# worldfnd/provekit

Hardware: AMD Instinct MI355X
Metric: proofs/sec (noir-r1cs prove hot path, WHIR commit + sumcheck + folding rounds) (higher is better)
Workload: dtype u32x8 (BN254-Fr, 256-bit Montgomery integers); 1 GPU; poseidon-rounds size class: m=21, m_0=20, satisfiable synthetic R1CS (786429 constraints, 1048571 witnesses, a constant term in half of the rows of A and B), batch-2 WHIR commit + zk-sumcheck + 4-round WHIR opening, queries [109, 28, 16, 11]/9, pow_bits [19.0, 16.0, 16.0, 18.0]/11.0 (WhirConfig::new derivation, security 128, ConjectureList), blinding WHIR n=8 queries [122]/31, Skyscraper-sponge tr; launcher=single process

## Files before the change

### provekit_amd/csrc/internal.hpp

```cpp
#pragma once
#include "ctx.hpp"
#include "rng_core.hpp"

namespace pk {

int ensure_scratch(pk_ctx* ctx, size_t bytes);
int ensure_pinned(pk_ctx* ctx);
int ensure_ws(pk_ctx* ctx, size_t bytes);
enum { PK_HOOK_GATE_SPINS = 0, PK_HOOK_GATE_STALL_US = 1, PK_HOOK_RCCL_SAME_DEVICE = 2, PK_HOOK_COUNT = 3 };
long test_hook(int which);
hipError_t wait_stream(int device, hipStream_t stream);
hipError_t wait_ctx(pk_ctx* ctx);
int wait_ctx_rc(pk_ctx* ctx);
int sync_stream(pk_ctx* ctx);
int mail_alloc(pk_ctx* ctx, size_t bytes, void** out);

int comm_rank(const pk_ctx* ctx);
int comm_world(const pk_ctx* ctx);
int comm_all_gather(pk_ctx* ctx, const void* d_send, void* d_recv, size_t bytes_per_rank);
int comm_all_reduce_sum_u64(pk_ctx* ctx, uint64_t* d_buf, size_t count);
int comm_collect_fe(pk_ctx* ctx, int K, uint64_t* host_out);
int red_across_begin(pk_ctx* ctx);
bool comm_collective_pending(const pk_ctx* ctx);
bool comm_rccl(const pk_ctx* ctx);
hipError_t comm_wait(pk_ctx* ctx);
void comm_turn_begin(pk_ctx* ctx);
void comm_turn_end(pk_ctx* ctx);
unsigned long long comm_collectives_issued(const pk_ctx* ctx);
void comm_abort(pk_ctx* ctx);
void comm_release(pk_ctx* ctx);

int leaf_hash_x(pk_ctx* ctx, const uint64_t* d_leaves, size_t n_leaves, size_t width, uint64_t* d_digests, bool scaled_in);
int merkle_top_x(pk_ctx* ctx, uint64_t* d_nodes, size_t top_leaves);
int read_root(pk_ctx* ctx, const uint64_t* d_nodes, size_t n_leaves, uint64_t root[4]);

void ntt_retain_ctx(pk_ctx* ctx);
void ntt_release_ctx(pk_ctx* ctx);
bool ntt_scaled_available(unsigned log_n);
int rs_encode_x(pk_ctx* ctx, const uint64_t* const* d_coeffs, unsigned batch, unsigned n_vars, unsigned log_inv_rate, unsigned fold,
                uint64_t* d_leaves, uint64_t* d_scratch, bool scaled);
int rs_encode_shard_x(pk_ctx* ctx, const uint64_t* const* d_coeffs, unsigned batch, unsigned n_vars, unsigned log_inv_rate, unsigned fold,
                      unsigned shard, unsigned n_shards, uint64_t* d_leaves_local, uint64_t* d_scratch, bool scaled);

int pow_solve_x(pk_ctx* ctx, const uint8_t challenge[32], double bits, uint64_t* nonce, bool striped);

unsigned shard_factor(const pk_ctx* ctx, size_t rows);
size_t commit_scratch_fes(const pk_ctx* ctx, size_t rows, size_t width);
int commit_into(pk_ctx* ctx, const uint64_t* const* d_coeffs, unsigned batch, unsigned n_vars, unsigned log_inv_rate, unsigned fold,
                uint64_t* d_leaves, uint64_t* d_nodes, uint64_t* d_scratch, pk_commit_layout* layout_out);
int open_raw(pk_ctx* ctx, const uint64_t* d_leaves, const uint64_t* d_nodes, size_t n_leaves, size_t width, const pk_commit_layout& lay,
             const uint64_t* indices, size_t k, int canonical_leaves, uint64_t* leaves_out, uint64_t* sibling_digests, uint64_t* auth_paths);

int eval_univariate_multi(pk_ctx* ctx, const uint64_t* const* d_polys, unsigned np, size_t n, const uint64_t z[4], uint64_t* out);
int dot_rows(pk_ctx* ctx, const uint64_t* d_w, size_t row_stride, unsigned nrows, const uint64_t* d_f, const uint64_t* d_g, size_t n, uint64_t* out,
             bool defer = false);
int lincomb2(pk_ctx* ctx, uint64_t* d_out, const uint64_t* d_a, const uint64_t* beta, const uint64_t* d_b, size_t n);
int fold_pairs2(pk_ctx* ctx, const uint64_t* d_v0, uint64_t* d_out0, const uint64_t* d_v1, uint64_t* d_out1, size_t len, const uint64_t* r,
                unsigned gate_seq = 0);
int sumcheck_cubic_launch(pk_ctx* ctx, uint64_t* d_a, uint64_t* d_b, uint64_t* d_c, uint64_t* d_eq, size_t len, const uint64_t* fold_or_null,
                          unsigned gate_seq, unsigned* red_seq_out);
int sumcheck_quadratic_launch(pk_ctx* ctx, const uint64_t* d_f, const uint64_t* d_w, size_t len, const uint64_t* fold_or_null, unsigned gate_seq,
                              uint64_t* d_f_out, uint64_t* d_w_out, int nsums, unsigned* red_seq_out);
void sumcheck_quadratic_from_claim(const uint64_t claim[4], uint64_t out[12]);
int eq_suffix_tables(pk_ctx* ctx, const uint64_t* r, unsigned n, uint64_t* d_out);
int sumcheck_cubic_spliteq_launch(pk_ctx* ctx, uint64_t* d_a, uint64_t* d_b, uint64_t* d_c, const uint64_t* d_level, size_t len,
                                  const uint64_t* fold_or_null, unsigned gate_seq, unsigned* red_seq_out);
void sumcheck_spliteq_correct(const uint64_t P[4], const uint64_t r_i[4], uint64_t out[12]);
void sumcheck_spliteq_advance(uint64_t P[4], const uint64_t r_i[4], const uint64_t alpha_i[4]);
int sumcheck_collect_spin(pk_ctx* ctx, int nsums, unsigned red_seq, uint64_t out[12]);
int sumcheck_collect(pk_ctx* ctx, int nsums, uint64_t out[12]);
unsigned sumcheck_gate_next(pk_ctx* ctx);
void sumcheck_gate_publish(pk_ctx* ctx, unsigned gate_seq, const uint64_t challenge[4]);
int sumcheck_gate_check(pk_ctx* ctx);
void sumcheck_gate_clear(pk_ctx* ctx);

int witness_bounds_strided(pk_ctx* ctx, const pk_r1cs* r, const uint64_t* d_z, unsigned m0, unsigned stride, unsigned offset, uint64_t* d_a,
                           uint64_t* d_b, uint64_t* d_c);
int external_row_range(pk_ctx* ctx, const pk_r1cs* r, const uint64_t* d_eq_alpha, size_t first, size_t last, uint64_t* d_out);

enum { RNG_MASK = 1, RNG_G = 2, RNG_BLIND = 3, RNG_MASK_B = 4, RNG_G_B = 5, RNG_FILL = 6 };
int proof_key(pk_ctx* ctx, const uint8_t* rng_seed32, RngKey& key);
int random_fe(pk_ctx* ctx, uint64_t* d_out, size_t n, const RngKey& key, uint32_t stream);

void witness_program_shape(const pk_witness_program* p, size_t* n_witnesses, size_t* n_challenges, size_t* n_acir);
int witness_phase_shape(const uint8_t* bytes, size_t len, std::vector<uint32_t>& widths, std::vector<uint32_t>& op_counts, std::vector<uint32_t>& blocks_before,
                        std::string& error);

const char* whir_config_error(const pk_whir_config* c);
unsigned blinding_log_len(unsigned m_0);
// ... 8 lines not shown
```

### provekit_amd/csrc/mle.hip

```cpp
#define PK_BASE_PRIO 2
#include "internal.hpp"
#include "fe29.hpp"
#include "reduce.hpp"

using namespace pk;

namespace {

struct fe_arg {
    u32 v[8];
};
__device__ __forceinline__ fe from_arg(const fe_arg& a) {
    fe r;
#pragma unroll
    for (int i = 0; i < 8; i++) r.v[i] = a.v[i];
    return r;
}
inline fe_arg to_arg(const uint64_t* h) {
    fe_arg a;
    memcpy(a.v, h, 32);
    return a;
}

__device__ __forceinline__ fe lds_get(const uint4* lo, const uint4* hi, int i) {
// ... 46 lines not shown
    const int R = 1 << logr;
    const int TILE = R * BT;
    uint4* lo = lds;
    uint4* hi = lds + TILE;
    const size_t vblocks = ((size_t)1 << s) / BT;
    const size_t u = blockIdx.x / vblocks, vb = blockIdx.x % vblocks;
    fe* base = data + (u << (s + logr)) + vb * BT;
    for (int e = threadIdx.x; e < TILE; e += 256) {
        int b = e % BT, r = e / BT;
        const uint4* q = reinterpret_cast<const uint4*>(base + ((size_t)r << s) + b);
        lo[e] = q[0];
        hi[e] = q[1];
    }
    __syncthreads();
    for (unsigned st = 0; st < logr; st++) {
        const int h = 1 << st;
        for (int t = threadIdx.x; t < (R / 2) * BT; t += 256) {
            int b = t % BT, j = t / BT;
            int pos = j & (h - 1);
            int i0 = ((j - pos) << 1) + pos, i1 = i0 + h;
            fe a = lds_get(lo, hi, i0 * BT + b), c = lds_get(lo, hi, i1 * BT + b);
            lds_put(lo, hi, i1 * BT + b, SUB ? fe_sub(c, a) : fe_add(c, a));
        }
        __syncthreads();
    }
    for (int e = threadIdx.x; e < TILE; e += 256) {
        int b = e % BT, r = e / BT;
        uint4* q = reinterpret_cast<uint4*>(base + ((size_t)r << s) + b);
        q[0] = lo[e];
        q[1] = hi[e];
    }
}

template <bool SUB>
int wavelet(pk_ctx* ctx, const uint64_t* d_src, uint64_t* d_data, unsigned n_vars) {
    PK_REQUIRE(ctx, d_data, "null pointer");
    PK_REQUIRE(ctx, n_vars <= 30, "too many variables");
    fe* D = (fe*)d_data;
    const fe* S = d_src ? (const fe*)d_src : D;
    if (n_vars == 0) {
        if (d_src && d_src != d_data) PK_HIP(ctx, hipMemcpyAsync(D, S, 32, hipMemcpyDeviceToDevice, ctx->stream));
        return PK_OK;
    }
    ProfScope prof(ctx, SUB ? "to_coeffs" : "to_evals");
    unsigned logt = n_vars < 11 ? n_vars : 11;
    size_t lds = ((size_t)2 << logt) * 16;
    PK_HIP(ctx, hipFuncSetAttribute((const void*)wavelet_low_kernel<SUB>, hipFuncAttributeMaxDynamicSharedMemorySize, 1 << 16));
    wavelet_low_kernel<SUB><<<(unsigned)((size_t)1 << (n_vars - logt)), 256, lds, ctx->stream>>>(S, D, logt);
    unsigned s = logt;
    PK_HIP(ctx, hipFuncSetAttribute((const void*)wavelet_high_kernel<SUB, 4>, hipFuncAttributeMaxDynamicSharedMemorySize, 1 << 16));
    PK_HIP(ctx, hipFuncSetAttribute((const void*)wavelet_high_kernel<SUB, 2>, hipFuncAttributeMaxDynamicSharedMemorySize, 1 << 16));
    while (s < n_vars) {
        unsigned left = n_vars - s;
        if (left == 10 && s >= 1) {
            size_t tiles = ((size_t)1 << (n_vars - 10)) / 2;
            wavelet_high_kernel<SUB, 2><<<(unsigned)tiles, 256, ((size_t)2 << 10) * 2 * 16, ctx->stream>>>(D, s, 10);
            s += 10;
        } else {
            unsigned logr = left < 9 ? left : 9;
            size_t tiles = ((size_t)1 << (n_vars - logr)) / 4;
            wavelet_high_kernel<SUB, 4><<<(unsigned)tiles, 256, ((size_t)2 << logr) * 4 * 16, ctx->stream>>>(D, s, logr);
            s += logr;
        }
    }
    PK_LAUNCH_CHECK(ctx);
    return PK_OK;
}

__global__ __launch_bounds__(256) void eq_half_tables_kernel(const fe* __restrict__ points, const fe* __restrict__ scales,
                                                             unsigned n_vars, unsigned nhi, unsigned nlo, fe* __restrict__ tables) {
    PK_LATENCY_PRIO();
    __shared__ uint4 xs[2 * 16];
    const unsigned pt = blockIdx.x, half = blockIdx.y;
    const size_t per_pt = ((size_t)1 << nhi) + ((size_t)1 << nlo);
    fe* T = tables + pt * per_pt + (half ? ((size_t)1 << nhi) : 0);
    const fe* x = points + (size_t)pt * n_vars + (half ? nhi : 0);
    const unsigned nv = half ? nlo : nhi;
    if (threadIdx.x < nv) lds_put(xs, xs + 16, threadIdx.x, fe_load(x + threadIdx.x));
    if (threadIdx.x == 32) fe_store(T, half ? fe_one() : fe_load(scales + pt));
    __threadfence_block();
    __syncthreads();
    for (unsigned l = 0; l < nv; l++) {
        const size_t h = (size_t)1 << l;
        fe xv = lds_get(xs, xs + 16, nv - 1 - l);
        for (size_t i = threadIdx.x; i < h; i += 256) {
            fe t = fe_load(T + i);
            fe up = fe_mulx(t, xv);
            fe_store(T + h + i, up);
            fe_store(T + i, fe_sub(t, up));
        }
        __threadfence_block();
        __syncthreads();
    }
}
__global__ __launch_bounds__(256) void eq_accumulate_kernel(fe* __restrict__ w, size_t n, unsigned nhi, unsigned nlo, unsigned q,
                                                            const fe* __restrict__ tables, int overwrite) {
    PK_LATENCY_PRIO();
    const size_t per_pt = ((size_t)1 << nhi) + ((size_t)1 << nlo);
    const size_t mask = ((size_t)1 << nlo) - 1;
// ... 466 lines not shown
#pragma unroll 1
            for (int j = 1; j < 16; j++) acc = fe_add(acc, fe_mulx(fe_load(c + t * 16 + j), lds_get(wts, wts + 16, j)));
            fe_store(out + t, acc);
        }
    } else {
        const size_t g = (size_t)blockIdx.x * blockDim.x + threadIdx.x, t = g >> 4;
        const unsigned j = threadIdx.x & 15;
        wide w = wide_zero();
        if (t < n_out) wide_add_fe(w, fe_mulx(fe_load(c + g), lds_get(wts, wts + 16, j)));
#pragma unroll
        for (unsigned off = 8; off >= 1; off >>= 1)
#pragma unroll
            for (int i = 0; i < 8; i++) w.l[i] += shfl_down_u64(w.l[i], off);
        if (j == 0 && t < n_out) fe_store(out + t, wide_reduce(w));
    }
}

__global__ __launch_bounds__(256) void lincomb_kernel(fe* __restrict__ out, const fe* __restrict__ a, const fe* __restrict__ b, size_t n,
                                                      fe_arg beta_arg) {
    PK_LATENCY_PRIO();
    const fe beta = from_arg(beta_arg);
    const size_t stride = (size_t)gridDim.x * blockDim.x;
    for (size_t i = (size_t)blockIdx.x * blockDim.x + threadIdx.x; i < n; i += stride)
        fe_store(out + i, fe_add(fe_load(a + i), fe_mulx(beta, fe_load(b + i))));
}
__global__ __launch_bounds__(256) void axpy_kernel(fe* __restrict__ y, const fe* __restrict__ x, size_t n, fe_arg beta_arg) {
    PK_LATENCY_PRIO();
    const fe beta = from_arg(beta_arg);
    const size_t stride = (size_t)gridDim.x * blockDim.x;
    for (size_t i = (size_t)blockIdx.x * blockDim.x + threadIdx.x; i < n; i += stride)
        fe_store(y + i, fe_add(fe_load(y + i), fe_mulx(beta, fe_load(x + i))));
}

int dot(pk_ctx* ctx, int nv, const uint64_t* d_w, const uint64_t* d_f, const uint64_t* d_g, size_t n, uint64_t* out) {
    if (n == 0) return reduce_empty(ctx, nv, out);
    red_out red;
    unsigned blocks;
    int rc = reduction_begin(ctx, n, &red, &blocks);
    if (rc) return rc;
    {
        ProfScope prof(ctx, "dot");
        auto kernel = nv == 2 ? dot_kernel<2> : dot_kernel<1>;
        kernel<<<blocks, RED_THREADS, 0, ctx->stream>>>((const fe*)d_w, (const fe*)d_f, (const fe*)d_g, n, red);
    }
    PK_LAUNCH_CHECK(ctx);
    return collect_reduction(ctx, nv, out);
}

}

namespace pk {

int sumcheck_cubic_launch(pk_ctx* ctx, uint64_t* d_a, uint64_t* d_b, uint64_t* d_c, uint64_t* d_eq, size_t len, const uint64_t* fold_or_null,
                          unsigned gate_seq, unsigned* red_seq_out) {
    PK_REQUIRE(ctx, d_a && d_b && d_c && d_eq && red_seq_out, "null pointer");
    PK_REQUIRE(ctx, is_pow2(len) && len >= 2, "size must be a power of two >= 2");
    const bool fold = fold_or_null || gate_seq;
    PK_REQUIRE(ctx, !fold || len >= 4, "size must be >= 4 when folding");
    const size_t npairs = fold ? len / 4 : len / 2;
    red_out red;
    unsigned blocks;
    int rc = reduction_begin(ctx, npairs, &red, &blocks);
    if (rc) return rc;
    *red_seq_out = red.seq;
    const gate_args gate = gate_seq ? gate_for(ctx, gate_seq) : gate_none();
    const fe_arg farg = fold_or_null ? to_arg(fold_or_null) : fe_arg{};
// ... 98 lines not shown
        ProfScope prof(ctx, "sumcheck_quadratic");
        kernel<<<blocks, RED_THREADS, 0, ctx->stream>>>((const fe*)d_f, (const fe*)d_w, out_len, farg, gate, (fe*)d_f_out, (fe*)d_w_out, red);
    }
    PK_LAUNCH_CHECK(ctx);
    return PK_OK;
}
int sumcheck_collect_spin(pk_ctx* ctx, int nsums, unsigned red_seq, uint64_t out[12]) { return collect_reduction_spin(ctx, nsums, red_seq, out); }
int sumcheck_collect(pk_ctx* ctx, int nsums, uint64_t out[12]) { return collect_reduction(ctx, nsums, out); }
void sumcheck_quadratic_from_claim(const uint64_t claim[4], uint64_t out[12]) {
    fe cl, h0;
    memcpy(cl.v, claim, 32);
    memcpy(h0.v, out, 32);
    const fe h1 = fe_sub(cl, h0);
    memcpy(out + 8, out + 4, 32);
    memcpy(out + 4, h1.v, 32);
}
unsigned sumcheck_gate_next(pk_ctx* ctx) { return gate_next(ctx); }
void sumcheck_gate_clear(pk_ctx* ctx) { (void)gate_timed_out(ctx); }
int sumcheck_gate_check(pk_ctx* ctx) { return gate_timed_out(ctx) ? set_err(ctx, PK_ERR_HIP, "%s", PK_GATE_TIMEOUT_MSG) : PK_OK; }
void sumcheck_gate_publish(pk_ctx* ctx, unsigned gate_seq, const uint64_t challenge[4]) {
    fe c;
    memcpy(c.v, challenge, 32);
    gate_publish(ctx, gate_seq, c);
}

int lincomb2(pk_ctx* ctx, uint64_t* d_out, const uint64_t* d_a, const uint64_t* beta, const uint64_t* d_b, size_t n) {
    PK_REQUIRE(ctx, beta && (n == 0 || (d_out && d_a && d_b)), "null pointer");
    if (!n) return PK_OK;
    ProfScope prof(ctx, "lincomb");
    lincomb_kernel<<<grid_for(ctx, n, 256), 256, 0, ctx->stream>>>((fe*)d_out, (const fe*)d_a, (const fe*)d_b, n, to_arg(beta));
    PK_LAUNCH_CHECK(ctx);
    return PK_OK;
}
int fold_pairs2(pk_ctx* ctx, const uint64_t* d_v0, uint64_t* d_out0, const uint64_t* d_v1, uint64_t* d_out1, size_t len, const uint64_t* r,
                unsigned gate_seq) {
    PK_REQUIRE(ctx, d_v0 && d_out0 && d_v1 && d_out1 && (r || gate_seq), "null pointer");
    PK_REQUIRE(ctx, is_pow2(len) && len >= 2, "size must be a power of two >= 2");
    if (gate_seq) {
        int rc = reduction_scratch(ctx);
        if (rc) return rc;
    }
    ProfScope prof(ctx, "fold_pairs");
    fold_pairs_kernel<<<dim3(grid_for(ctx, len / 2, 256), 2), 256, 0, ctx->stream>>>((const fe*)d_v0, (fe*)d_out0, (const fe*)d_v1, (fe*)d_out1,
                                                                                     len / 2, r ? to_arg(r) : fe_arg{},
                                                                                     gate_seq ? gate_for(ctx, gate_seq) : gate_none());
    PK_LAUNCH_CHECK(ctx);
    return PK_OK;
}

int eval_univariate_multi(pk_ctx* ctx, const uint64_t* const* d_polys, unsigned np, size_t n, const uint64_t z[4], uint64_t* out) {
    PK_REQUIRE(ctx, np == 1 || np == 2, "one or two polynomials");
    if (n == 0) return reduce_empty(ctx, (int)np, out);
    PK_REQUIRE(ctx, (n >> 28) == 0, "polynomial too long for the evaluation kernel (2^28 coefficients)");
    red_out red;
    unsigned blocks;
    int rc = reduction_begin(ctx, n, &red, &blocks);
    if (rc) return rc;
    size_t want = (n / 8 + RED_THREADS - 1) / RED_THREADS;
    const size_t cap = want < 1 ? 1 : (want > RED_MAX_BLOCKS ? RED_MAX_BLOCKS : want);
    const size_t cnt = (n + cap * RED_THREADS - 1) / (cap * RED_THREADS);
    blocks = (unsigned)((n + cnt * RED_THREADS - 1) / (cnt * RED_THREADS));
    if (!ctx->d_ztab) PK_HIP(ctx, hipMalloc(&ctx->d_ztab, 256 * 32));
    pow2_args zp;
    {
        fe b;
        memcpy(b.v, z, 32);
// ... 221 lines not shown
```

### provekit_amd/csrc/prover.hip

```cpp
#include <unistd.h>

#include <algorithm>
#include <chrono>
#include <cstdlib>
#include <string>
#include <vector>

#include "internal.hpp"
#include "shard_map.hpp"
#include "prover_transcript.hpp"

using namespace pk;

struct pk_scheme {
    const pk_r1cs* r1cs = nullptr;
    size_t num_constraints = 0, num_witnesses = 0;
    unsigned m = 0, m_0 = 0;
    unsigned nb = 0;
    pk_whir_config whir_witness{}, whir_hiding{};
    char* arena = nullptr;
    size_t arena_bytes = 0;
    std::string domain_separator;
    char* noir_witness = nullptr;
    pk_ctx* side = nullptr;
// ... 198 lines not shown
    C.nodes = nodes;
    CK(ensure_ws(ctx, commit_scratch_fes(ctx, C.rows, C.width) * 32));
    const uint64_t* ptrs[4];
    for (unsigned b = 0; b < batch; b++) ptrs[b] = U(polys[b]);
    return commit_into(ctx, ptrs, batch, n_vars, log_inv_rate, fold, U(leaves), U(nodes), (uint64_t*)ctx->d_ws, &C.layout);
}
int whir_commit_transcript(pk_ctx* ctx, const pk_whir_config& cfg, const fe& root, Transcript& T, Commitment& C) {
    const unsigned batch = C.batch;
    fe* const* polys = C.polys;
    T.add_canon(root);
    C.ood_points.resize(cfg.commitment_ood_samples);
    T.challenge_scalars(C.ood_points.data(), C.ood_points.size());
    C.ood_answers.resize((size_t)batch * C.ood_points.size());
    for (size_t j = 0; j < C.ood_points.size(); j++) {
        for (unsigned b = 0; b < batch; b += 2) {
            const unsigned np = batch - b >= 2 ? 2 : 1;
            fe ans[2];
            CK(eval_univariate_multi_x(ctx, polys + b, np, (size_t)1 << cfg.n_vars, C.ood_points[j], ans));
            for (unsigned q = 0; q < np; q++) C.ood_answers[(b + q) * C.ood_points.size() + j] = ans[q];
        }
    }
    for (unsigned b = 0; b < batch; b++) T.add_scalars(&C.ood_answers[b * C.ood_points.size()], C.ood_points.size());
    C.beta = batch > 1 ? T.challenge_scalar() : fe_one();
    return PK_OK;
}

bool whir_sharded(const pk_ctx* ctx, unsigned n_vars) {
    const size_t G = (size_t)comm_world(ctx);
    return G > 1 && (((size_t)1 << n_vars) / G) >= 2 * SHARD_MIN_LOCAL;
}
size_t in_block(size_t stored, size_t off, size_t len) {
    const size_t hi = stored < off + len ? stored : off + len;
    return hi > off ? hi - off : 0;
}
struct WhirProver {
    pk_ctx* ctx;
    Arena& A;
    const pk_whir_config& cfg;
    const Commitment& C;
    Transcript& T;
    const unsigned n, k, G, lgG, rank;
    bool sharded;
    const size_t B0, off0;
    fe* d_c = nullptr;
    fe* bp[2] = {};
    fe* bw[2] = {};
    fe* gathered[4] = {};
    int cur = 0;
    size_t len;
    std::vector<fe> rs;
    fe claim;
    bool have_claim = false;
    std::vector<fe> all_r;

    WhirProver(pk_ctx* c, Arena& a, const pk_whir_config& cf, const Commitment& com, Transcript& t)
        : ctx(c), A(a), cfg(cf), C(com), T(t), n(cf.n_vars), k(cf.folding_factor), G((unsigned)comm_world(c)), lgG(ilog2(G)),
          rank((unsigned)comm_rank(c)), sharded(whir_sharded(c, n)), B0(sharded ? ((size_t)1 << n) / G : (size_t)1 << n),
          off0(sharded ? (size_t)rank * B0 : 0), len(B0) {}

    int batch_combine(fe* dst, fe* const* x, size_t from, size_t cnt) {
        if (C.batch == 1) return pk_memcpy_d2d(ctx, dst, x[0] + from, 32 * cnt);
        uint64_t s[4];
        h_store(s, C.beta);
        int rc = lincomb2(ctx, U(dst), U(x[0] + from), s, U(x[1] + from), cnt);
        fe bp_ = h_mul(C.beta, C.beta);
        for (unsigned b = 2; b < C.batch && !rc; b++) {
// ... 61 lines not shown
            const fe msg[3] = {h_load(out), h_load(out + 4), h_load(out + 8)};
            T.add_scalars(msg, 3);
            const fe r = T.challenge_scalar();
            gate.publish(r);
            rs.push_back(r);
            all_r.push_back(r);
            claim = eval_quadratic_012(msg, r);
            have_claim = true;
        }
        if (!pipelined && rounds && len >= 2) {
            uint64_t f[4];
            h_store(f, rs.back());
            CK(fold_pairs2(ctx, U(bp[cur]), U(bp[1 - cur]), U(bw[cur]), U(bw[1 - cur]), len, f));
            flip();
        }
        return PK_OK;
    }

    int gather(fe* p0, fe* p1, fe* w0, fe* w1) {
        CK(gather_blocks(ctx, bp[cur], len, p0));
        CK(gather_blocks(ctx, bw[cur], len, w0));
        bp[0] = p0; bp[1] = p1; bw[0] = w0; bw[1] = w1;
        cur = 0;
        len *= G;
        sharded = false;
        return PK_OK;
    }
    int maybe_gather() { return sharded && len <= SHARD_MIN_LOCAL ? gather(gathered[0], gathered[1], gathered[2], gathered[3]) : PK_OK; }

    int start(fe* const* d_weights, const size_t* weight_len, unsigned n_weights, const fe* weight_sums) {
        const size_t N = (size_t)1 << n;
        ALLOC(dc, N);
        d_c = dc;
        CK(batch_combine(d_c, C.polys, 0, N));
        ALLOC(p0, B0);
        ALLOC(p1, B0 / 2 ? B0 / 2 : 1);
        ALLOC(w0, B0);
        ALLOC(w1, B0 / 2 ? B0 / 2 : 1);
        bp[0] = p0; bp[1] = p1; bw[0] = w0; bw[1] = w1;
        bool have_evals = true;
        for (unsigned b = 0; b < C.batch; b++) have_evals = have_evals && C.evals[b] != nullptr;
        if (have_evals) {
            CK(batch_combine(p0, C.evals, off0, B0));
        } else if (!sharded) {
            CK(pk_to_evals_into(ctx, U(d_c), U(p0), n));
        } else {
            ALLOC(d_ev, N);
            CK(pk_to_evals_into(ctx, U(d_c), U(d_ev), n));
            CK(pk_memcpy_d2d(ctx, p0, d_ev + off0, 32 * B0));
        }
        const fe gamma = T.challenge_scalar();
        fe g;
        CK(eq_weights(w0, n, C.ood_points, gamma, 1, &g));
        auto batched = [&](const fe* v, size_t step) {
            fe acc = v[0], bb = C.beta;
            for (unsigned b = 1; b < C.batch; b++, bb = h_mul(bb, C.beta)) acc = h_add(acc, h_mul(bb, v[b * step]));
            return acc;
        };
        const size_t q = C.ood_points.size();
        claim = fe_zero();
        fe gq = fe_one();
        for (size_t j = 0; j < q; j++, gq = h_mul(gq, gamma)) claim = h_add(claim, h_mul(gq, batched(&C.ood_answers[j], q)));
        have_claim = weight_sums || !n_weights;
        for (unsigned i = 0; i < n_weights; i++) {
            uint64_t s[4];
            h_store(s, g);
            const size_t cnt = in_block(weight_len[i], off0, B0);
            if (cnt) CK(pk_fe_axpy(ctx, U(w0), s, U(d_weights[i] + off0), cnt));
            if (weight_sums) claim = h_add(claim, h_mul(g, batched(weight_sums + (size_t)i * C.batch, 1)));
            g = h_mul(g, gamma);
        }
        if (sharded) {
            const size_t cap = G * SHARD_MIN_LOCAL;
            const size_t sizes[4] = {cap, cap / 2, cap, cap / 2};
            for (int q = 0; q < 4; q++) {
                ALLOC(buf, sizes[q]);
                gathered[q] = buf;
            }
        }
        CK(sumcheck_rounds(k));
        return maybe_gather();
    }

    int rounds() {
        const Commitment* prev = &C;
        Commitment com;
        unsigned nv = n, log_inv_rate = cfg.starting_log_inv_rate;
        size_t domain_size = (size_t)1 << (n + log_inv_rate);
        fe exp_gen = folded_domain_generator(n + log_inv_rate, k);
        for (unsigned r = 0; r < cfg.n_rounds; r++) {
            const unsigned nv2 = nv - k;
            ALLOC(d_c2, (size_t)1 << nv2);
            CK(pk_fold_coeffs(ctx, U(d_c), nv, (const uint64_t*)rs.data(), k, U(d_c2)));
            d_c = d_c2;
            nv = nv2;
            log_inv_rate += k - 1;
            Commitment next;
            CK(whir_commit_compute(ctx, A, nv, log_inv_rate, k, &d_c, 1, next));
            fe root;
            CK(read_root(ctx, U(next.nodes), next.rows, (uint64_t*)root.v));
            T.add_canon(root);
// ... 26 lines not shown
            ALLOC(fp0, cap);
            ALLOC(fp1, cap / 2 ? cap / 2 : 1);
            ALLOC(fw0, cap);
            ALLOC(fw1, cap / 2 ? cap / 2 : 1);
            CK(gather(fp0, fp1, fw0, fw1));
        }
        const unsigned nv2 = nv - k;
        ALLOC(d_final, (size_t)1 << nv2);
        CK(pk_fold_coeffs(ctx, U(d_c), nv, (const uint64_t*)rs.data(), k, U(d_final)));
        std::vector<fe> fin((size_t)1 << nv2);
        CK(pk_memcpy_d2h(ctx, fin.data(), d_final, 32 * fin.size()));
        T.add_scalars(fin.data(), fin.size());
        CK(pow_round(ctx, T, cfg.final_pow_bits));
        const std::vector<uint64_t> idx = stir_queries(T, domain_size, k, cfg.final_queries);
        CK(emit_opening_hints(ctx, T, prev, idx));
        CK(sumcheck_rounds(nv2));
        return pow_round(ctx, T, cfg.final_folding_pow_bits);
    }

    int deferred_hint(fe* const* d_weights, const size_t* weight_len, unsigned n_weights) {
        if (!n_weights) return PK_OK;
        std::vector<fe> point(all_r.rbegin(), all_r.rend());
        const bool sh = whir_sharded(ctx, n);
        ALLOC(d_eq, B0);
        if (sh) {
            const fe sc = eq_bits(point.data(), lgG, rank);
            CK(pk_eq_accumulate(ctx, U(d_eq), n - lgG, (const uint64_t*)(point.data() + lgG), (const uint64_t*)&sc, 1, 1));
        } else {
            CK(pk_eq_table(ctx, (const uint64_t*)point.data(), n, U(d_eq)));
        }
        Across ac(ctx, sh);
        CK(ac.rc);
        std::vector<fe> evals(n_weights);
        const bool rows3 = n_weights == 3 && weight_len[0] == weight_len[1] && weight_len[1] == weight_len[2] && d_weights[1] > d_weights[0] &&
                           d_weights[1] - d_weights[0] == d_weights[2] - d_weights[1];
        if (rows3) {
            uint64_t o[12] = {};
            if (sh || weight_len[0])
                CK(dot_rows(ctx, U(d_weights[0] + off0), (size_t)(d_weights[1] - d_weights[0]), 3, U(d_eq), nullptr, in_block(weight_len[0], off0, B0), o));
            for (int i = 0; i < 3; i++) evals[i] = h_load(o + 4 * i);
        } else {
            for (unsigned i = 0; i < n_weights; i++) {
                uint64_t o[4] = {};
                if (sh || weight_len[i]) CK(pk_dot(ctx, U(d_weights[i] + off0), U(d_eq), in_block(weight_len[i], off0, B0), o));
                evals[i] = h_load(o);
            }
        }
        std::vector<uint8_t> buf;
        put_vec(buf, evals.data(), n_weights);
        T.hint(buf.data(), buf.size());
        return PK_OK;
    }
};
int whir_prove(pk_ctx* ctx, Arena& A, const pk_whir_config& cfg, const Commitment& C, fe* const* d_weights, const size_t* weight_len,
               unsigned n_weights, const fe* weight_sums, Transcript& T) {
    WhirProver P(ctx, A, cfg, C, T);
    CK(P.start(d_weights, weight_len, n_weights, weight_sums));
    CK(P.rounds());
    return P.deferred_hint(d_weights, weight_len, n_weights);
}

struct BatchCommit {
    Commitment com;
    fe* f_evals = nullptr;
    fe* g_evals = nullptr;
};
int batch_commit_compute(pk_ctx* ctx, Arena& A, unsigned m, const pk_whir_config& cfg, const fe* d_evals, size_t n_evals, const RngKey& key,
                         u32 stream_mask, u32 stream_g, BatchCommit& out) {
    const size_t half = (size_t)1 << (m - 1), N = 2 * half;
    ALLOC(f, N);
    ALLOC(g, N);
    ALLOC(fe_, N);
    ALLOC(ge_, N);
    CK(pk_memset_zero(ctx, f, 32 * half));
    CK(pk_memcpy_d2d(ctx, f, d_evals, 32 * n_evals));
    {
        ProfScope prof(ctx, "random_fe");
        CK(random_fe(ctx, U(f + half), half, key, stream_mask));
        CK(random_fe(ctx, U(g), N, key, stream_g));
    }
    CK(pk_to_coeffs_into(ctx, U(f), U(fe_), m));
    CK(pk_to_coeffs_into(ctx, U(g), U(ge_), m));
    out.f_evals = f;
    out.g_evals = g;
    fe* polys[2] = {fe_, ge_};
    int rc = whir_commit_compute(ctx, A, cfg.n_vars, cfg.starting_log_inv_rate, cfg.folding_factor, polys, 2, out.com);
    out.com.evals[0] = f;
    out.com.evals[1] = g;
    return rc;
}

__global__ void gather_fe_kernel(const fe* __restrict__ src, const uint32_t* __restrict__ idx, size_t n, fe* __restrict__ dst) {
    const size_t i = (size_t)blockIdx.x * blockDim.x + threadIdx.x;
    if (i < n) fe_store(dst + i, fe_load(src + idx[i]));
}

struct AbortOnFailure {
    pk_ctx* c;
    unsigned long long issued0;
    int rc = PK_ERR_HIP;
    explicit AbortOnFailure(pk_ctx* ctx) : c(ctx), issued0(comm_collectives_issued(ctx)) {}
    int done(int status) { return rc = status; }
    ~AbortOnFailure() {
        if (rc == PK_OK) return;
        struct Drain {
            pk_ctx* c;
            ~Drain() {
                (void)wait_ctx(c);
                sumcheck_gate_clear(c);
            }
        } drain{c};
        if (comm_world(c) <= 1) return;
        const bool same_everywhere = rc == PK_ERR_BAD_ARG || rc == PK_ERR_UNSATISFIED || rc == PK_ERR_IO_PATTERN;
        if (comm_rccl(c) && same_everywhere && comm_collectives_issued(c) == issued0) return;
        comm_abort(c);
// ... 455 lines not shown
```

### provekit_amd/csrc/rng.hip

```cpp
#include <sys/random.h>

#include <cerrno>

#include "internal.hpp"
#include "fe29.hpp"

using namespace pk;

namespace {

__global__ __launch_bounds__(256) void random_fe_kernel(fe* __restrict__ out, size_t n, RngKey key, u32 stream) {
    PK_LATENCY_PRIO();
    const size_t stride = (size_t)gridDim.x * blockDim.x, pairs = (n + 1) / 2;
    size_t j = (size_t)blockIdx.x * blockDim.x + threadIdx.x;
    u32 attempt = 0;
    bool done0 = false, done1 = 2 * j + 1 >= n;
    while (j < pairs) {
        u32 blk[16];
        chacha_block(key, (u64)j, stream, attempt, PK_RNG_ROUNDS, blk);
#pragma unroll
        for (int half = 0; half < 2; half++) {
            if (half == 0 ? done0 : done1) continue;
            fe x;
            if (rng_candidate(blk, half, x)) {
                fe_store(out + 2 * j + half, x);
                if (half == 0) done0 = true;
                else done1 = true;
            }
        }
        if (done0 && done1) {
            j += stride;
            attempt = 0;
            done0 = false;
            done1 = 2 * j + 1 >= n;
        } else {
            attempt++;
        }
    }
}
inline unsigned random_fe_grid(const pk_ctx* ctx, size_t n) {
    const size_t pairs = (n + 1) / 2;
    size_t blocks = (pairs + 256 * 8 - 1) / (256 * 8);
    const size_t cap = (size_t)ctx->num_cus * 8;
    if (blocks < 1) blocks = 1;
    return (unsigned)(blocks < cap ? blocks : cap);
}

__global__ __launch_bounds__(256) void fill_witness_kernel(fe* __restrict__ w, const uint8_t* __restrict__ is_set, size_t n, RngKey key, u32 stream,
                                                           unsigned long long* n_filled) {
    PK_LATENCY_PRIO();
    const size_t stride = (size_t)gridDim.x * blockDim.x;
    unsigned mine = 0;
    for (size_t i = (size_t)blockIdx.x * blockDim.x + threadIdx.x; i < n; i += stride) {
        if (is_set[i]) continue;
        u32 blk[16];
        chacha_block(key, (u64)(i >> 2), stream, 0, PK_RNG_ROUNDS, blk);
        fe x = fe_zero();
#pragma unroll
        for (int k = 0; k < 4; k++) {
            u32 v = 0;
#pragma unroll
            for (int q = 0; q < 4; q++) v = (i & 3) == (size_t)q ? blk[4 * q + k] : v;
            x.v[k] = v;
        }
        fe_store(w + i, fe_to_montx(x));
        mine++;
    }
    if (mine) atomicAdd(n_filled, (unsigned long long)mine);
}

}
// ... 84 lines not shown
```

### provekit_amd/csrc/rng_core.hpp

```cpp
#pragma once
#include "fe.hpp"

namespace pk {

struct RngKey {
    uint32_t k[8];
};

enum { PKW_RNG_MASK0 = 16, PKW_RNG_G = 24 };

constexpr int PK_RNG_ROUNDS = 12;
#define PK_QR(a, b, c, d)                    \
    a += b; d ^= a; d = (d << 16) | (d >> 16); \
    c += d; b ^= c; b = (b << 12) | (b >> 20); \
    a += b; d ^= a; d = (d << 8) | (d >> 24);  \
    c += d; b ^= c; b = (b << 7) | (b >> 25)
__host__ __device__ __forceinline__ void chacha_block(const RngKey& key, u64 counter, u32 n0, u32 n1, int rounds, u32 (&out)[16]) {
    u32 s[16] = {0x61707865u, 0x3320646eu, 0x79622d32u, 0x6b206574u, key.k[0], key.k[1], key.k[2], key.k[3],
                 key.k[4],    key.k[5],    key.k[6],    key.k[7],    (u32)counter, (u32)(counter >> 32), n0, n1};
    u32 x[16];
#pragma unroll
    for (int i = 0; i < 16; i++) x[i] = s[i];
#pragma unroll 1
    for (int r = 0; r < rounds / 2; r++) {
        PK_QR(x[0], x[4], x[8], x[12]);
        PK_QR(x[1], x[5], x[9], x[13]);
        PK_QR(x[2], x[6], x[10], x[14]);
        PK_QR(x[3], x[7], x[11], x[15]);
        PK_QR(x[0], x[5], x[10], x[15]);
        PK_QR(x[1], x[6], x[11], x[12]);
        PK_QR(x[2], x[7], x[8], x[13]);
        PK_QR(x[3], x[4], x[9], x[14]);
    }
#pragma unroll
    for (int i = 0; i < 16; i++) out[i] = x[i] + s[i];
}
#undef PK_QR

__host__ __device__ __forceinline__ bool rng_candidate(const u32 (&blk)[16], int half, fe& x) {
#pragma unroll
    for (int w = 0; w < 8; w++) x.v[w] = blk[8 * half + w];
    x.v[7] &= 0x3fffffffu;
    u32 borrow = 0;
#pragma unroll
    for (int k = 0; k < 8; k++) (void)__builtin_subc(x.v[k], kPlimb(k), borrow, &borrow);
    return borrow != 0;
}

}
```

Measured before the change: 283.8 proofs/s.

## Fuse mask generation into wavelet pass and batch lincomb/axpy launches

Adds a fused kernel that copies the witness, draws ChaCha-based random field elements directly into LDS and the eval buffers, and runs the low wavelet stages in one pass for both f and g tables. This replaces the separate memset, memcpy, two random_fe launches and two low wavelet kernels on single-GPU runs. It also merges the two batch_combine calls into a paired lincomb kernel and the three weight axpys into one axpy3 kernel that reads the three rows together. These changes cut launches and global memory round-trips, at the cost of more specialised code paths that only apply to batch-2 and equal-stride-3 layouts.

```diff
diff --git a/provekit_amd/csrc/internal.hpp b/provekit_amd/csrc/internal.hpp
--- a/provekit_amd/csrc/internal.hpp
+++ b/provekit_amd/csrc/internal.hpp
@@ -55,6 +55,11 @@
 int dot_rows(pk_ctx* ctx, const uint64_t* d_w, size_t row_stride, unsigned nrows, const uint64_t* d_f, const uint64_t* d_g, size_t n, uint64_t* out,
              bool defer = false);
 int lincomb2(pk_ctx* ctx, uint64_t* d_out, const uint64_t* d_a, const uint64_t* beta, const uint64_t* d_b, size_t n);
+int lincomb2_pair(pk_ctx* ctx, uint64_t* d_out0, const uint64_t* d_a0, const uint64_t* d_b0, size_t n0, uint64_t* d_out1, const uint64_t* d_a1,
+                  const uint64_t* d_b1, size_t n1, const uint64_t* beta);
+int axpy3(pk_ctx* ctx, uint64_t* d_y, const uint64_t* g3, const uint64_t* d_rows, size_t row_stride, size_t n);
+int to_coeffs_generated(pk_ctx* ctx, unsigned m, const uint64_t* d_wit, size_t n_wit, const RngKey& key, uint32_t stream_mask, uint32_t stream_g,
+                        uint64_t* d_f_evals, uint64_t* d_g_evals, uint64_t* d_f_coeffs, uint64_t* d_g_coeffs);
 int fold_pairs2(pk_ctx* ctx, const uint64_t* d_v0, uint64_t* d_out0, const uint64_t* d_v1, uint64_t* d_out1, size_t len, const uint64_t* r,
                 unsigned gate_seq = 0);
 int sumcheck_cubic_launch(pk_ctx* ctx, uint64_t* d_a, uint64_t* d_b, uint64_t* d_c, uint64_t* d_eq, size_t len, const uint64_t* fold_or_null,
diff --git a/provekit_amd/csrc/mle.hip b/provekit_amd/csrc/mle.hip
--- a/provekit_amd/csrc/mle.hip
+++ b/provekit_amd/csrc/mle.hip
@@ -102,22 +102,65 @@
     }
 }
 
+struct gen_table {
+    const fe* wit;
+    size_t n_wit, rand_from, n_draw;
+    u32 stream;
+    fe* evals;
+    fe* coeffs;
+};
+__global__ __launch_bounds__(256) void wavelet_low_generated_kernel(gen_table ta, gen_table tb, RngKey key, unsigned logt) {
+    PK_LATENCY_PRIO();
+    extern __shared__ uint4 lds[];
+    const gen_table& S = blockIdx.y ? tb : ta;
+    const int T = 1 << logt;
+    uint4* lo = lds;
+    uint4* hi = lds + T;
+    const size_t t0 = (size_t)blockIdx.x * T;
+    for (int e = threadIdx.x; e < T && t0 + e < S.rand_from; e += 256) {
+        uint4 a = make_uint4(0, 0, 0, 0), b = a;
+        if (t0 + e < S.n_wit) {
+            const uint4* q = reinterpret_cast<const uint4*>(S.wit + t0 + e);
+            a = q[0];
+            b = q[1];
+        }
+        lo[e] = a;
+        hi[e] = b;
+        uint4* o = reinterpret_cast<uint4*>(S.evals + t0 + e);
+        o[0] = a;
+        o[1] = b;
+    }
+    if (t0 + T > S.rand_from) {
+        const size_t d0 = (t0 > S.rand_from ? t0 : S.rand_from) - S.rand_from, d1 = t0 + T - S.rand_from;
+        fe* ev = S.evals + S.rand_from;
+        const size_t shift = S.rand_from - t0;
+        rng_draw_pairs(key, S.stream, d0 / 2 + threadIdx.x, 256, (d1 + 1) / 2, S.n_draw, [&](size_t i, const fe& x) {
+            fe_store(ev + i, x);
+            lds_put(lo, hi, (int)(i + shift), x);
+        });
+    }
+    __syncthreads();
+    for (unsigned s = 0; s < logt; s++) {
+        const int h = 1 << s;
+        for (int t = threadIdx.x; t < T / 2; t += 256) {
+            int pos = t & (h - 1);
+            int i0 = ((t - pos) << 1) + pos, i1 = i0 + h;
+            fe a = lds_get(lo, hi, i0), b = lds_get(lo, hi, i1);
+            lds_put(lo, hi, i1, fe_sub(b, a));
+        }
+        __syncthreads();
+    }
+    fe* base = S.coeffs + t0;
+    for (int e = threadIdx.x; e < T; e += 256) {
+        uint4* q = reinterpret_cast<uint4*>(base + e);
+        q[0] = lo[e];
+        q[1] = hi[e];
+    }
+}
+
+inline unsigned wavelet_low_bits(unsigned n_vars) { return n_vars < 11 ? n_vars : 11; }
 template <bool SUB>
-int wavelet(pk_ctx* ctx, const uint64_t* d_src, uint64_t* d_data, unsigned n_vars) {
-    PK_REQUIRE(ctx, d_data, "null pointer");
-    PK_REQUIRE(ctx, n_vars <= 30, "too many variables");
-    fe* D = (fe*)d_data;
-    const fe* S = d_src ? (const fe*)d_src : D;
-    if (n_vars == 0) {
-        if (d_src && d_src != d_data) PK_HIP(ctx, hipMemcpyAsync(D, S, 32, hipMemcpyDeviceToDevice, ctx->stream));
-        return PK_OK;
-    }
-    ProfScope prof(ctx, SUB ? "to_coeffs" : "to_evals");
-    unsigned logt = n_vars < 11 ? n_vars : 11;
-    size_t lds = ((size_t)2 << logt) * 16;
-    PK_HIP(ctx, hipFuncSetAttribute((const void*)wavelet_low_kernel<SUB>, hipFuncAttributeMaxDynamicSharedMemorySize, 1 << 16));
-    wavelet_low_kernel<SUB><<<(unsigned)((size_t)1 << (n_vars - logt)), 256, lds, ctx->stream>>>(S, D, logt);
-    unsigned s = logt;
+int wavelet_high_sweeps(pk_ctx* ctx, fe* D, unsigned s, unsigned n_vars) {
     PK_HIP(ctx, hipFuncSetAttribute((const void*)wavelet_high_kernel<SUB, 4>, hipFuncAttributeMaxDynamicSharedMemorySize, 1 << 16));
     PK_HIP(ctx, hipFuncSetAttribute((const void*)wavelet_high_kernel<SUB, 2>, hipFuncAttributeMaxDynamicSharedMemorySize, 1 << 16));
     while (s < n_vars) {
@@ -135,6 +178,24 @@
     }
     PK_LAUNCH_CHECK(ctx);
     return PK_OK;
+}
+
+template <bool SUB>
+int wavelet(pk_ctx* ctx, const uint64_t* d_src, uint64_t* d_data, unsigned n_vars) {
+    PK_REQUIRE(ctx, d_data, "null pointer");
+    PK_REQUIRE(ctx, n_vars <= 30, "too many variables");
+    fe* D = (fe*)d_data;
+    const fe* S = d_src ? (const fe*)d_src : D;
+    if (n_vars == 0) {
+        if (d_src && d_src != d_data) PK_HIP(ctx, hipMemcpyAsync(D, S, 32, hipMemcpyDeviceToDevice, ctx->stream));
+        return PK_OK;
+    }
+    ProfScope prof(ctx, SUB ? "to_coeffs" : "to_evals");
+    const unsigned logt = wavelet_low_bits(n_vars);
+    size_t lds = ((size_t)2 << logt) * 16;
+    PK_HIP(ctx, hipFuncSetAttribute((const void*)wavelet_low_kernel<SUB>, hipFuncAttributeMaxDynamicSharedMemorySize, 1 << 16));
+    wavelet_low_kernel<SUB><<<(unsigned)((size_t)1 << (n_vars - logt)), 256, lds, ctx->stream>>>(S, D, logt);
+    return wavelet_high_sweeps<SUB>(ctx, D, logt, n_vars);
 }
 
 __global__ __launch_bounds__(256) void eq_half_tables_kernel(const fe* __restrict__ points, const fe* __restrict__ scales,
@@ -667,6 +728,36 @@
         fe_store(y + i, fe_add(fe_load(y + i), fe_mulx(beta, fe_load(x + i))));
 }
 
+__global__ __launch_bounds__(256) void lincomb_pair_kernel(fe* __restrict__ out0, const fe* __restrict__ a0, const fe* __restrict__ b0, size_t n0,
+                                                           fe* __restrict__ out1, const fe* __restrict__ a1, const fe* __restrict__ b1, size_t n1,
+                                                           fe_arg beta_arg) {
+    PK_LATENCY_PRIO();
+    const fe beta = from_arg(beta_arg);
+    fe* out = blockIdx.y ? out1 : out0;
+    const fe* a = blockIdx.y ? a1 : a0;
+    const fe* b = blockIdx.y ? b1 : b0;
+    const size_t n = blockIdx.y ? n1 : n0;
+    const size_t stride = (size_t)gridDim.x * blockDim.x;
+    for (size_t i = (size_t)blockIdx.x * blockDim.x + threadIdx.x; i < n; i += stride)
+        fe_store(out + i, fe_add(fe_load(a + i), fe_mulx(beta, fe_load(b + i))));
+}
+struct fe3_arg {
+    fe_arg g[3];
+};
+__global__ __launch_bounds__(256) void axpy3_kernel(fe* __restrict__ y, const fe* __restrict__ rows, size_t row_stride, size_t n, fe3_arg ga) {
+    PK_LATENCY_PRIO();
+    const fe29 g0 = unpack29<5>(from_arg(ga.g[0])), g1 = unpack29<5>(from_arg(ga.g[1])), g2 = unpack29<5>(from_arg(ga.g[2]));
+    const size_t stride = (size_t)gridDim.x * blockDim.x;
+    for (size_t i = (size_t)blockIdx.x * blockDim.x + threadIdx.x; i < n; i += stride) {
+        dot29 d;
+        dot29_init(d);
+        dot29_add(d, unpack29<0>(fe_load(rows + i)), g0);
+        dot29_add(d, unpack29<0>(fe_load(rows + row_stride + i)), g1);
+        dot29_add(d, unpack29<0>(fe_load(rows + 2 * row_stride + i)), g2);
+        fe_store(y + i, fe_add(fe_load(y + i), dot29_result(d)));
+    }
+}
+
 int dot(pk_ctx* ctx, int nv, const uint64_t* d_w, const uint64_t* d_f, const uint64_t* d_g, size_t n, uint64_t* out) {
     if (n == 0) return reduce_empty(ctx, nv, out);
     red_out red;
@@ -831,6 +922,40 @@
     PK_LAUNCH_CHECK(ctx);
     return PK_OK;
 }
+int lincomb2_pair(pk_ctx* ctx, uint64_t* d_out0, const uint64_t* d_a0, const uint64_t* d_b0, size_t n0, uint64_t* d_out1, const uint64_t* d_a1,
+                  const uint64_t* d_b1, size_t n1, const uint64_t* beta) {
+    PK_REQUIRE(ctx, beta && (n0 == 0 || (d_out0 && d_a0 && d_b0)) && (n1 == 0 || (d_out1 && d_a1 && d_b1)), "null pointer");
+    if (!n0 && !n1) return PK_OK;
+    ProfScope prof(ctx, "lincomb");
+    lincomb_pair_kernel<<<dim3(grid_for(ctx, n0 > n1 ? n0 : n1, 256), 2), 256, 0, ctx->stream>>>(
+        (fe*)d_out0, (const fe*)d_a0, (const fe*)d_b0, n0, (fe*)d_out1, (const fe*)d_a1, (const fe*)d_b1, n1, to_arg(beta));
+    PK_LAUNCH_CHECK(ctx);
+    return PK_OK;
+}
+int axpy3(pk_ctx* ctx, uint64_t* d_y, const uint64_t* g3, const uint64_t* d_rows, size_t row_stride, size_t n) {
+    PK_REQUIRE(ctx, g3 && (n == 0 || (d_y && d_rows)), "null pointer");
+    if (!n) return PK_OK;
+    ProfScope prof(ctx, "lincomb");
+    fe3_arg ga;
+    for (int k = 0; k < 3; k++) ga.g[k] = to_arg(g3 + 4 * k);
+    axpy3_kernel<<<grid_for(ctx, n, 256), 256, 0, ctx->stream>>>((fe*)d_y, (const fe*)d_rows, row_stride, n, ga);
+    PK_LAUNCH_CHECK(ctx);
+    return PK_OK;
+}
+int to_coeffs_generated(pk_ctx* ctx, unsigned m, const uint64_t* d_wit, size_t n_wit, const RngKey& key, uint32_t stream_mask, uint32_t stream_g,
+                        uint64_t* d_f_evals, uint64_t* d_g_evals, uint64_t* d_f_coeffs, uint64_t* d_g_coeffs) {
+    PK_REQUIRE(ctx, d_f_evals && d_g_evals && d_f_coeffs && d_g_coeffs && (n_wit == 0 || d_wit), "null pointer");
+    PK_REQUIRE(ctx, m >= 1 && m <= 30 && n_wit <= ((size_t)1 << (m - 1)), "witness longer than half the table");
+    const size_t half = (size_t)1 << (m - 1), N = 2 * half;
+    const gen_table tf = {(const fe*)d_wit, n_wit, half, half, stream_mask, (fe*)d_f_evals, (fe*)d_f_coeffs};
+    const gen_table tg = {nullptr, 0, 0, N, stream_g, (fe*)d_g_evals, (fe*)d_g_coeffs};
+    ProfScope prof(ctx, "to_coeffs");
+    const unsigned logt = wavelet_low_bits(m);
+    PK_HIP(ctx, hipFuncSetAttribute((const void*)wavelet_low_generated_kernel, hipFuncAttributeMaxDynamicSharedMemorySize, 1 << 16));
+    wavelet_low_generated_kernel<<<dim3((unsigned)(N >> logt), 2), 256, ((size_t)2 << logt) * 16, ctx->stream>>>(tf, tg, key, logt);
+    int rc = wavelet_high_sweeps<true>(ctx, (fe*)d_f_coeffs, logt, m);
+    return rc ? rc : wavelet_high_sweeps<true>(ctx, (fe*)d_g_coeffs, logt, m);
+}
 int fold_pairs2(pk_ctx* ctx, const uint64_t* d_v0, uint64_t* d_out0, const uint64_t* d_v1, uint64_t* d_out1, size_t len, const uint64_t* r,
                 unsigned gate_seq) {
     PK_REQUIRE(ctx, d_v0 && d_out0 && d_v1 && d_out1 && (r || gate_seq), "null pointer");
diff --git a/provekit_amd/csrc/prover.hip b/provekit_amd/csrc/prover.hip
--- a/provekit_amd/csrc/prover.hip
+++ b/provekit_amd/csrc/prover.hip
@@ -254,6 +254,10 @@
 size_t in_block(size_t stored, size_t off, size_t len) {
     const size_t hi = stored < off + len ? stored : off + len;
     return hi > off ? hi - off : 0;
+}
+bool rows_at_equal_stride3(fe* const* d_weights, const size_t* weight_len, unsigned n_weights) {
+    return n_weights == 3 && weight_len[0] == weight_len[1] && weight_len[1] == weight_len[2] && d_weights[1] > d_weights[0] &&
+           d_weights[1] - d_weights[0] == d_weights[2] - d_weights[1];
 }
 struct WhirProver {
     pk_ctx* ctx;
@@ -381,7 +385,6 @@
         const size_t N = (size_t)1 << n;
         ALLOC(dc, N);
         d_c = dc;
-        CK(batch_combine(d_c, C.polys, 0, N));
         ALLOC(p0, B0);
         ALLOC(p1, B0 / 2 ? B0 / 2 : 1);
         ALLOC(w0, B0);
@@ -389,8 +392,16 @@
         bp[0] = p0; bp[1] = p1; bw[0] = w0; bw[1] = w1;
         bool have_evals = true;
         for (unsigned b = 0; b < C.batch; b++) have_evals = have_evals && C.evals[b] != nullptr;
+        const bool pair = have_evals && C.batch == 2;
+        if (pair) {
+            uint64_t s[4];
+            h_store(s, C.beta);
+            CK(lincomb2_pair(ctx, U(d_c), U(C.polys[0]), U(C.polys[1]), N, U(p0), U(C.evals[0] + off0), U(C.evals[1] + off0), B0, s));
+        } else {
+            CK(batch_combine(d_c, C.polys, 0, N));
+        }
         if (have_evals) {
-            CK(batch_combine(p0, C.evals, off0, B0));
+            if (!pair) CK(batch_combine(p0, C.evals, off0, B0));
         } else if (!sharded) {
             CK(pk_to_evals_into(ctx, U(d_c), U(p0), n));
         } else {
@@ -411,11 +422,18 @@
         fe gq = fe_one();
         for (size_t j = 0; j < q; j++, gq = h_mul(gq, gamma)) claim = h_add(claim, h_mul(gq, batched(&C.ood_answers[j], q)));
         have_claim = weight_sums || !n_weights;
+        const bool rows3 = rows_at_equal_stride3(d_weights, weight_len, n_weights);
+        if (rows3) {
+            uint64_t s3[12];
+            fe g3 = g;
+            for (int i = 0; i < 3; i++, g3 = h_mul(g3, gamma)) h_store(s3 + 4 * i, g3);
+            CK(axpy3(ctx, U(w0), s3, U(d_weights[0] + off0), (size_t)(d_weights[1] - d_weights[0]), in_block(weight_len[0], off0, B0)));
+        }
         for (unsigned i = 0; i < n_weights; i++) {
             uint64_t s[4];
             h_store(s, g);
             const size_t cnt = in_block(weight_len[i], off0, B0);
-            if (cnt) CK(pk_fe_axpy(ctx, U(w0), s, U(d_weights[i] + off0), cnt));
+            if (cnt && !rows3) CK(pk_fe_axpy(ctx, U(w0), s, U(d_weights[i] + off0), cnt));
             if (weight_sums) claim = h_add(claim, h_mul(g, batched(weight_sums + (size_t)i * C.batch, 1)));
             g = h_mul(g, gamma);
         }
@@ -508,8 +526,7 @@
         Across ac(ctx, sh);
         CK(ac.rc);
         std::vector<fe> evals(n_weights);
-        const bool rows3 = n_weights == 3 && weight_len[0] == weight_len[1] && weight_len[1] == weight_len[2] && d_weights[1] > d_weights[0] &&
-                           d_weights[1] - d_weights[0] == d_weights[2] - d_weights[1];
+        const bool rows3 = rows_at_equal_stride3(d_weights, weight_len, n_weights);
         if (rows3) {
             uint64_t o[12] = {};
             if (sh || weight_len[0])
@@ -548,15 +565,19 @@
     ALLOC(g, N);
     ALLOC(fe_, N);
     ALLOC(ge_, N);
-    CK(pk_memset_zero(ctx, f, 32 * half));
-    CK(pk_memcpy_d2d(ctx, f, d_evals, 32 * n_evals));
-    {
-        ProfScope prof(ctx, "random_fe");
-        CK(random_fe(ctx, U(f + half), half, key, stream_mask));
-        CK(random_fe(ctx, U(g), N, key, stream_g));
-    }
-    CK(pk_to_coeffs_into(ctx, U(f), U(fe_), m));
-    CK(pk_to_coeffs_into(ctx, U(g), U(ge_), m));
+    if (comm_world(ctx) <= 1) {
+        CK(to_coeffs_generated(ctx, m, U(d_evals), n_evals, key, stream_mask, stream_g, U(f), U(g), U(fe_), U(ge_)));
+    } else {
+        CK(pk_memset_zero(ctx, f, 32 * half));
+        CK(pk_memcpy_d2d(ctx, f, d_evals, 32 * n_evals));
+        {
+            ProfScope prof(ctx, "random_fe");
+            CK(random_fe(ctx, U(f + half), half, key, stream_mask));
+            CK(random_fe(ctx, U(g), N, key, stream_g));
+        }
+        CK(pk_to_coeffs_into(ctx, U(f), U(fe_), m));
+        CK(pk_to_coeffs_into(ctx, U(g), U(ge_), m));
+    }
     out.f_evals = f;
     out.g_evals = g;
     fe* polys[2] = {fe_, ge_};
diff --git a/provekit_amd/csrc/rng.hip b/provekit_amd/csrc/rng.hip
--- a/provekit_amd/csrc/rng.hip
+++ b/provekit_amd/csrc/rng.hip
@@ -11,32 +11,8 @@
 
 __global__ __launch_bounds__(256) void random_fe_kernel(fe* __restrict__ out, size_t n, RngKey key, u32 stream) {
     PK_LATENCY_PRIO();
-    const size_t stride = (size_t)gridDim.x * blockDim.x, pairs = (n + 1) / 2;
-    size_t j = (size_t)blockIdx.x * blockDim.x + threadIdx.x;
-    u32 attempt = 0;
-    bool done0 = false, done1 = 2 * j + 1 >= n;
-    while (j < pairs) {
-        u32 blk[16];
-        chacha_block(key, (u64)j, stream, attempt, PK_RNG_ROUNDS, blk);
-#pragma unroll
-        for (int half = 0; half < 2; half++) {
-            if (half == 0 ? done0 : done1) continue;
-            fe x;
-            if (rng_candidate(blk, half, x)) {
-                fe_store(out + 2 * j + half, x);
-                if (half == 0) done0 = true;
-                else done1 = true;
-            }
-        }
-        if (done0 && done1) {
-            j += stride;
-            attempt = 0;
-            done0 = false;
-            done1 = 2 * j + 1 >= n;
-        } else {
-            attempt++;
-        }
-    }
+    rng_draw_pairs(key, stream, (size_t)blockIdx.x * blockDim.x + threadIdx.x, (size_t)gridDim.x * blockDim.x, (n + 1) / 2, n,
+                   [&](size_t i, const fe& x) { fe_store(out + i, x); });
 }
 inline unsigned random_fe_grid(const pk_ctx* ctx, size_t n) {
     const size_t pairs = (n + 1) / 2;
diff --git a/provekit_amd/csrc/rng_core.hpp b/provekit_amd/csrc/rng_core.hpp
--- a/provekit_amd/csrc/rng_core.hpp
+++ b/provekit_amd/csrc/rng_core.hpp
@@ -47,4 +47,33 @@
     return borrow != 0;
 }
 
+template <class Put>
+__device__ __forceinline__ void rng_draw_pairs(const RngKey& key, u32 stream, size_t first, size_t stride, size_t pairs_end, size_t n, Put put) {
+    size_t j = first;
+    u32 attempt = 0;
+    bool done0 = false, done1 = 2 * j + 1 >= n;
+    while (j < pairs_end) {
+        u32 blk[16];
+        chacha_block(key, (u64)j, stream, attempt, PK_RNG_ROUNDS, blk);
+#pragma unroll
+        for (int half = 0; half < 2; half++) {
+            if (half == 0 ? done0 : done1) continue;
+            fe x;
+            if (rng_candidate(blk, half, x)) {
+                put(2 * j + half, x);
+                if (half == 0) done0 = true;
+                else done1 = true;
+            }
+        }
+        if (done0 && done1) {
+            j += stride;
+            attempt = 0;
+            done0 = false;
+            done1 = 2 * j + 1 >= n;
+        } else {
+            attempt++;
+        }
+    }
 }
+
+}
```

Result: faster. 292.5 proofs/s (median of 6 runs) (+3.1%).
